# sulaimanvesal/PointCloudUDA

Hardware: AMD Instinct MI355X
Metric: adversarial train-step images/sec (seg+3 discr) at 256x256 (higher is better)
Workload: dtype bf16x3 MFMA (split-bf16, fp32 accumulate; fp32 storage); 1 GPU; MS-CMRSeg full UDA: UNet(PointNet head) + d1 + d2 + d4, 256x256x1, 4 classes; per_gpu_batch=32, global_batch=32, precision=bf16x3, parallelism=dp1, ranks_in_group=1, collective=none, streams=discriminators concurrent, d_target_forward=replayed from the adversarial pass of the same step, launch=eager (256 host cores for this rank)

## Files before the change

pointcloududa_amd/csrc/conv_wgrad.hip:

```cpp
#include "conv_igemm.h"
#include "conv_host.h"

struct ReduceJobs {
  int n;
  int first_block[PCUDA_REDUCE_MAX_JOBS + 1];
  pcuda_reduce_job j[PCUDA_REDUCE_MAX_JOBS];
};

__global__ __launch_bounds__(1024) void wgrad_reduce_batch_kernel(const ReduceJobs jobs) {
  __shared__ float sh[16][64];
  int lo = 0, hi = jobs.n - 1;
  while (lo < hi) {
    const int mid = (lo + hi + 1) >> 1;
    if (jobs.first_block[mid] <= (int)blockIdx.x) lo = mid; else hi = mid - 1;
  }
  const pcuda_reduce_job& jb = jobs.j[lo];
  const float* partial = jb.partial;
  long long numel = jb.numel;
  float* dw = jb.dw;
  int ntaps = jb.ntaps;
  const int ksplit = jb.ksplit, nkg = jb.nkg;
  const int lane = threadIdx.x & 63, kg = threadIdx.x >> 6;
  const long long nblk_w = (numel + 63) / 64;
  long long blk = (int)blockIdx.x - jobs.first_block[lo];
  if (blk >= nblk_w) { blk -= nblk_w; partial = jb.db_partial; numel = jb.nb; dw = jb.db; ntaps = 1; }
  const long long i = blk * 64 + lane;
  float s = 0.f;
  if (i < numel && kg < nkg) {
    int k = kg;
    for (; k + 7 * nkg < ksplit; k += 8 * nkg) {
      float v[8];
#pragma unroll
      for (int u = 0; u < 8; ++u) v[u] = partial[(long long)(k + u * nkg) * numel + i];
#pragma unroll
      for (int u = 0; u < 8; ++u) s += v[u];
    }
    for (; k < ksplit; k += nkg) s += partial[(long long)k * numel + i];
  }
  sh[kg][lane] = s;
  __syncthreads();
  if (kg == 0 && i < numel) {
    float t = 0.f;
    for (int q = 0; q < nkg; ++q) t += sh[q][lane];
    long long o = i;
    if (ntaps > 1) {
      const long long cc = numel / ntaps;
      const long long tt = i / cc, r = i - tt * cc;
      o = r * ntaps + tt;
    }
    dw[o] = jb.accumulate ? dw[o] + t : t;
  }
}

static int reduce_blocks(const pcuda_reduce_job& jb) { return cdiv(jb.numel, 64) + (jb.db ? cdiv(jb.nb, 64) : 0); }

static int launch_reduce_jobs(const ReduceJobs& jobs, int threads, hipStream_t s) {
  hipLaunchKernelGGL(wgrad_reduce_batch_kernel, dim3(jobs.first_block[jobs.n]), dim3(threads), 0, s, jobs);
  PCUDA_CHECK_LAUNCH("wgrad_reduce_batch_kernel");
  return PCUDA_OK;
}

static pcuda_reduce_job reduce_job(const float* partial, long long numel, int ksplit, float* dw, int accumulate, int ntaps,
                                   const float* db_partial, long long nb, float* db) {
  pcuda_reduce_job jb;
  memset(&jb, 0, sizeof(jb));
  jb.partial = partial; jb.numel = numel; jb.ksplit = ksplit; jb.dw = dw; jb.accumulate = accumulate; jb.ntaps = ntaps;
  jb.db_partial = db_partial; jb.nb = db ? nb : 0; jb.db = db;
  jb.nkg = 1;
  while (jb.nkg < 16 && jb.nkg * 2 <= ksplit) jb.nkg <<= 1;
  return jb;
}

static int launch_reduce_job(const pcuda_reduce_job& jb, hipStream_t s) {
  ReduceJobs jobs;
  jobs.n = 1;
  jobs.j[0] = jb;
  jobs.first_block[0] = 0;
  jobs.first_block[1] = reduce_blocks(jb);
  return launch_reduce_jobs(jobs, 64 * jb.nkg, s);
}
int launch_wgrad_reduce(const float* partial, long long numel, int ksplit, float* dw, int accumulate, int ntaps,
                        const float* db_partial, long long nb, float* db, hipStream_t s) {
  return launch_reduce_job(reduce_job(partial, numel, ksplit, dw, accumulate, ntaps, db_partial, nb, db), s);
}

WgradSlabs wgrad_slabs(const WgradCall& c, int slices, int ntaps) {
  WgradSlabs sl;
  sl.welems = (long long)c.g->cout * c.g->cin * c.g->k * c.g->k;
  sl.partial = (float*)c.workspace;
  sl.db_partial = c.db ? sl.partial + (size_t)slices * sl.welems : nullptr;
  sl.slices = slices; sl.ntaps = ntaps;
  return sl;
}

int wgrad_finish(const WgradCall& c, const WgradSlabs& sl) {
  const pcuda_reduce_job jb = reduce_job(sl.partial, sl.welems, sl.slices, c.dw, c.accumulate, sl.ntaps, sl.db_partial, c.g->cout, c.db);
  if (!c.defer) return launch_reduce_job(jb, c.s);
  *c.defer = jb;
  return PCUDA_OK;
}

extern "C" int pcuda_wgrad_reduce_batch(const pcuda_reduce_job* host_jobs, int njobs, pcuda_stream_t s) {
  if (!host_jobs || njobs < 0) PCUDA_FAIL(PCUDA_E_BADARG, "wgrad_reduce_batch: bad arguments");
  int done = 0;
  while (done < njobs) {
    ReduceJobs jobs;
    jobs.n = 0;
    int blocks = 0;
    for (; done < njobs && jobs.n < PCUDA_REDUCE_MAX_JOBS; ++done) {
      const pcuda_reduce_job& jb = host_jobs[done];
      if (jb.ksplit <= 0) continue;
      if (!jb.partial || !jb.dw || jb.numel <= 0 || jb.nkg < 1 || jb.nkg > 16 || (jb.db && !jb.db_partial))
        PCUDA_FAIL(PCUDA_E_BADARG, "wgrad_reduce_batch: bad job %d", done);
      jobs.first_block[jobs.n] = blocks;
      jobs.j[jobs.n++] = jb;
      blocks += reduce_blocks(jb);
    }
    if (jobs.n == 0) break;
    jobs.first_block[jobs.n] = blocks;
    ProfScope prof(PCUDA_FAM_POINTWISE, 0.0, (hipStream_t)s, "wgrad reduce batch");
    const int rc = launch_reduce_jobs(jobs, 1024, (hipStream_t)s);
    if (rc) return rc;
  }
  return PCUDA_OK;
}

namespace {

struct WgradPlan {
  int co_blks, co_tile, n_co_tiles, n_chunks, tap_groups, taps_per_group, tw, th, tiles_x, tiles_y, ksplit;
  int ih_t, iw_t;
};

struct TileSpan {
  long long halo, clipped;
};
TileSpan tile_span(const pcuda_conv_geom* g, long long ih, long long iw) {
  return {ih * iw, (ih < g->in_h ? ih : g->in_h) * (iw < g->in_w ? iw : g->in_w) + 1};
}
size_t stage_lds(long long x_pixels, int co_tile, size_t mul) {
  return (size_t)x_pixels * IG_REC_BYTES * mul + (size_t)co_tile * WG_ZROW * mul;
}

struct WgradStage {
  bool clamp;
  int x_cap;
  size_t lds;
};
WgradStage wgrad_stage(const WgradPlan& w, const pcuda_conv_geom* g, size_t mul) {
  const TileSpan t = tile_span(g, w.ih_t, w.iw_t);
  WgradStage st;
  st.clamp = t.clipped * 2 <= t.halo || stage_lds(t.halo, w.co_tile, mul) > (size_t)LDS_HARD;
  st.x_cap = (int)(st.clamp ? t.clipped : t.halo);
  st.lds = stage_lds(st.x_cap, w.co_tile, mul);
  return st;
}

WgradPlan plan_wgrad(const pcuda_conv_geom* g) {
  WgradPlan w;
  w.co_blks = ig_co_blks(g->cout);
  w.co_tile = 32 * w.co_blks;
  w.n_co_tiles = cdiv(g->cout, w.co_tile);
  w.n_chunks = cdiv(g->cin, 32);
  const int ntaps = g->k * g->k;
  w.tap_groups = ntaps <= 16 ? 1 : cdiv(ntaps, 9);
  w.taps_per_group = cdiv(ntaps, w.tap_groups);
  const int span = (g->k - 1) * g->dil;
  {
    int cand[16];
    const int nc = tile_width_candidates(g->out_w, 128, cand);
    long long best_key = -1;
    w.tw = 32; w.th = 4;
    for (int ci = 0; ci < nc; ++ci) {
      const int tw = cand[ci], th = 128 / tw;
      if (th < 1) continue;
      const TileSpan t = tile_span(g, (th - 1) * g->stride + span + 1, (tw - 1) * g->stride + span + 1);
      const long long cap = t.halo < t.clipped ? t.halo : t.clipped;
      if (stage_lds(cap, w.co_tile, 2) > (size_t)LDS_HARD) continue;
      const long long staged = (t.clipped * 2 <= t.halo) ? t.clipped : t.halo;
      const long long key = ((long long)cdiv(g->out_w, tw) * cdiv(g->out_h, th) << 24) + (staged > 768 ? (1ll << 22) : 0) +
                            ((tw & 31) ? (1ll << 20) : 0) + t.halo;
      if (best_key < 0 || key < best_key) { best_key = key; w.tw = tw; w.th = th; }
    }
  }
  const int TW = w.tw, TH = w.th;
  w.tiles_x = cdiv(g->out_w, TW);
  w.tiles_y = cdiv(g->out_h, TH);
  w.ih_t = (TH - 1) * g->stride + span + 1;
  w.iw_t = (TW - 1) * g->stride + span + 1;
  const long long ntiles = (long long)g->n * w.tiles_x * w.tiles_y;
  const int base = w.n_co_tiles * w.n_chunks * w.tap_groups;
  static const int tgt32 = env_knob("PCUDA_WG_BLOCKS32", 768);
  static const int tgt64 = env_knob("PCUDA_WG_BLOCKS64", 1024);
  static const int tgt1 = env_knob("PCUDA_WG_BLOCKS1", 256);
  const bool one_per_cu = wgrad_stage(w, g, 2).lds > (size_t)LDS_HARD / 2;
  long long ks = (one_per_cu ? tgt1 : (w.co_blks == 1 ? tgt32 : tgt64)) / base;
  if (ks < 1) ks = 1;
  if (ks > ntiles) ks = ntiles;
  const long long welems = (long long)g->cout * g->cin * ntaps;
  while (ks > 1 && ks * welems * 4 > (64ll << 20)) ks >>= 1;
  if (ks >= 8) ks &= ~7ll;
  w.ksplit = (int)ks;
  return w;
}

int wgrad_prefetch(const WgradCall& c, const WgradPlan& w, int x_cap) {
  static const bool nopipe = env_knob("PCUDA_NOPIPE", 0) != 0;
  int pf = (nopipe || !fast_src_ok(c.x, c.g->cin)) ? 0 : (x_cap <= 256 ? 1 : (x_cap <= 768 ? 3 : 0));
  static const bool now8 = env_knob("PCUDA_WG_NO8", 0) != 0;
  if (!now8 && pf > 0 && w.taps_per_group > 9 && x_cap <= 1024) pf = 100 + (x_cap <= 512 ? 1 : 2);
  return pf;
}

WgradParams wgrad_params(const WgradCall& c, const WgradPlan& w, const TapSet& t, const WgradStage& st, int pf, const dim3& grid) {
  const pcuda_conv_geom* g = c.g;
  WgradParams p;
  memset(&p, 0, sizeof(p));
  p.x = *c.x; p.cin = g->cin;
  p.in_h = g->in_h; p.in_w = g->in_w; p.in_shift = g->in_up ? 1 : 0; p.in_row = g->in_w >> p.in_shift;
  p.dz = c.dy; p.dz_sn = c.dy_sn; p.dz_sc = c.dy_sc;
  p.cout = g->cout; p.out_h = g->out_h; p.out_w = g->out_w;
  p.stride = g->stride;
  p.ntaps = w.taps_per_group; p.ntaps_total = t.n; p.tap_groups = w.tap_groups;
  memcpy(p.dy, t.dy, sizeof(p.dy));
  memcpy(p.dx, t.dx, sizeof(p.dx));
  p.dy_min = t.dy_min; p.dx_min = t.dx_min;
  p.ih_t = w.ih_t; p.iw_t = w.iw_t;
  p.tw = w.tw; p.th = w.th; p.tmagic = 65536 / w.tw + 1; p.tiles_x = w.tiles_x; p.tiles_y = w.tiles_y; p.n = g->n;
  p.ksplit = w.ksplit; p.n_co_tiles = w.n_co_tiles; p.n_chunks = w.n_chunks;
  p.partial = (float*)c.workspace;
  static const int dbg = env_knob("PCUDA_DBG", 0);
  p.dbg = dbg;
  p.tw16 = ((w.tw & 15) == 0 && w.tw * w.th == 128) ? 1 : 0;
  p.aligned4 = ((g->out_w & 7) == 0 && (w.tw & 7) == 0 && aligned16(c.dy, c.dy_sn, c.dy_sc) &&
                ((long long)g->cout * c.dy_sc + (long long)g->out_h * g->out_w) * 4 < (1ll << 30)) ? 1 : 0;
  static const bool noxcd = env_knob("PCUDA_WG_NOXCD", 0) != 0;
  static const bool nointer = env_knob("PCUDA_WG_NOINTER", 0) != 0;
  const long long nblk = (long long)grid.x * grid.y;
  p.xcd_items = (!noxcd && nblk >= 16 && (nblk & 7) == 0) ? (int)(nblk / 8) : 0;
  p.xcd_slices = (p.xcd_items && !nointer && (w.ksplit & 7) == 0) ? w.ksplit / 8 : 0;
  {
    static const bool noxq = env_knob("PCUDA_NOXQ", 0) != 0;
    const int slots = pf >= 100 ? pf - 100 : pf, per = pf >= 100 ? 128 : 64;
    const int ih = st.clamp ? (w.ih_t < g->in_h ? w.ih_t : g->in_h) : w.ih_t;
    const int in_w_phys = g->in_up ? g->in_w / 2 : g->in_w;
    p.xq = (!noxq && slots > 0 && !g->in_up && (in_w_phys & 3) == 0 && (ih * ((w.iw_t + 6) / 4) + per - 1) / per <= slots) ? 1 : 0;
  }
  return p;
}

}

int wgrad_dispatch_x3(const WgradParams& p, int co_blks, bool clamp, int taps_max, int pf, int x_cap, size_t lds,
                      float* dbp, dim3 grid, hipStream_t s);
int wgrad_dispatch_bf16(const WgradParams& p, int co_blks, bool clamp, int taps_max, int pf, int x_cap, size_t lds,
                        float* dbp, dim3 grid, hipStream_t s);

static int generic_slices(const pcuda_conv_geom* g) { return plan_wgrad(g).ksplit; }
static int generic_wgrad(const WgradCall& c) {
  const pcuda_conv_geom* g = c.g;
  const bool x3 = c.prec == PCUDA_PREC_BF16X3;
  const WgradPlan w = plan_wgrad(g);
  const TapSet t = fwd_taps(g);
  const WgradSlabs sl = wgrad_slabs(c, w.ksplit, t.n);
  const WgradStage st = wgrad_stage(w, g, x3 ? 2 : 1);
  if (st.lds > (size_t)LDS_HARD) PCUDA_FAIL(PCUDA_E_UNSUPPORTED, "conv2d_wgrad: tile %dx%d does not fit LDS", w.ih_t, w.iw_t);
  const dim3 grid(w.n_co_tiles * w.n_chunks * w.tap_groups, w.ksplit);
  const int pf = wgrad_prefetch(c, w, st.x_cap);
  const WgradParams p = wgrad_params(c, w, t, st, pf, grid);
  {
    const double flops = 2.0 * g->n * (double)g->out_h * g->out_w * g->cout * (double)g->cin * t.n;
    char tag[160];
    snprintf(tag, sizeof(tag), "wgrad n%d cin%d cout%d %dx%d k%d s%d d%d ksplit%d clamp%d pf%d lds%zu", g->n, g->cin,
             g->cout, g->out_h, g->out_w, g->k, g->stride, g->dil, w.ksplit, st.clamp ? 1 : 0, pf, st.lds);
    ProfScope prof(PCUDA_FAM_CONV_WGRAD, flops, c.s, tag);
    const int taps_max = w.taps_per_group <= 1 ? 1 : w.taps_per_group <= 9 ? 9 : 16;
    const int rc = x3 ? wgrad_dispatch_x3(p, w.co_blks, st.clamp, taps_max, pf, st.x_cap, st.lds, sl.db_partial, grid, c.s)
                      : wgrad_dispatch_bf16(p, w.co_blks, st.clamp, taps_max, pf, st.x_cap, st.lds, sl.db_partial, grid, c.s);
    if (rc) return rc;
  }
  return wgrad_finish(c, sl);
}

struct WgradRoute {
  const char* name;
  int (*slices)(const pcuda_conv_geom* g);
  size_t (*bytes)(const pcuda_conv_geom* g);
  int (*run)(const WgradCall& c);
};
static const WgradRoute WGRAD_ROUTES[] = {
    {"direct c1", direct_wgrad_slices, nullptr, direct_wgrad},
    {"direct d1", nullptr, direct_d1_wgrad_bytes, direct_d1_wgrad},
    {"wgrad3r", wgrad3r_slices, nullptr, wgrad3r_wgrad},
    {"wgrad3", wgrad3_slices, nullptr, wgrad3_wgrad},
    {"wgrad1", wgrad1_slices, nullptr, wgrad1_wgrad},
    {"generic", generic_slices, nullptr, generic_wgrad},
};

extern "C" size_t pcuda_conv2d_wgrad_workspace_size(const pcuda_conv_geom* g) {
  if (!geom_ok(g)) return 0;
  size_t need = 0;
  for (const WgradRoute& r : WGRAD_ROUTES) {
    size_t b = 0;
    if (r.bytes) b = r.bytes(g);
    else if (const int slices = r.slices(g)) b = wgrad_slab_bytes(g, slices);
    if (b > need) need = b;
  }
  return need;
}

static int wgrad_impl(const WgradCall& c, size_t workspace_bytes) {
  const pcuda_conv_geom* g = c.g;
  if (!geom_ok(g)) PCUDA_FAIL(PCUDA_E_BADARG, "conv2d_wgrad: inconsistent geometry");
  if (!src_ok(c.x, g->cin) || !c.dy || !c.dw) PCUDA_FAIL(PCUDA_E_BADARG, "conv2d_wgrad: bad tensors");
  if (c.prec != PCUDA_PREC_BF16X3 && c.prec != PCUDA_PREC_BF16) PCUDA_FAIL(PCUDA_E_BADARG, "conv2d_wgrad: bad precision");
  if (!c.workspace || workspace_bytes < pcuda_conv2d_wgrad_workspace_size(g))
    PCUDA_FAIL(PCUDA_E_WORKSPACE, "conv2d_wgrad: workspace too small (%zu < %zu)", workspace_bytes,
               pcuda_conv2d_wgrad_workspace_size(g));
  for (const WgradRoute& r : WGRAD_ROUTES) {
    const int rc = r.run(c);
    if (rc != WGRAD_NOT_TAKEN) return rc;
  }
  PCUDA_FAIL(PCUDA_E_UNSUPPORTED, "conv2d_wgrad: no route took the layer");
}

extern "C" int pcuda_conv2d_wgrad(const pcuda_conv_geom* g, int prec, const pcuda_src* x, const float* dy,
                                  long long dy_sn, long long dy_sc, float* dw, float* db, int accumulate,
                                  void* workspace, size_t workspace_bytes, pcuda_stream_t s) {
  return wgrad_impl({g, prec, x, dy, dy_sn, dy_sc, dw, db, accumulate, workspace, (hipStream_t)s, nullptr}, workspace_bytes);
}

extern "C" int pcuda_conv2d_wgrad_partial(const pcuda_conv_geom* g, int prec, const pcuda_src* x, const float* dy,
                                          long long dy_sn, long long dy_sc, float* dw, float* db, int accumulate,
                                          void* workspace, size_t workspace_bytes, pcuda_reduce_job* job, pcuda_stream_t s) {
  if (!job) PCUDA_FAIL(PCUDA_E_BADARG, "conv2d_wgrad_partial: job is NULL");
  memset(job, 0, sizeof(*job));
  return wgrad_impl({g, prec, x, dy, dy_sn, dy_sc, dw, db, accumulate, workspace, (hipStream_t)s, job}, workspace_bytes);
}
```

pointcloududa_amd/csrc/dense.hip:

```cpp
#include "common.h"

struct GemmParams {
  const float* a; long long a_sb, a_si, a_sl;
  const float* b; long long b_sb, b_sl, b_sj;
  float* c; long long c_sb, c_si, c_sj;
  const float* bias;
  int m, n, k, accumulate;
};

#define GT 32
__global__ __launch_bounds__(256) void gemm_kernel(const GemmParams p) {
  __shared__ float As[GT][GT + 1], Bs[GT][GT + 1];
  const int bz = blockIdx.z;
  const float* A = p.a + bz * p.a_sb;
  const float* B = p.b + bz * p.b_sb;
  float* C = p.c + bz * p.c_sb;
  const int i0 = blockIdx.y * GT, j0 = blockIdx.x * GT;
  const int tj = threadIdx.x & 31, ti = threadIdx.x >> 5;
  float acc[4] = {0.f, 0.f, 0.f, 0.f};
  for (int l0 = 0; l0 < p.k; l0 += GT) {
    for (int e = threadIdx.x; e < GT * GT; e += 256) {
      const int r = e >> 5, cc = e & 31;
      int ia, la;
      if (p.a_sl == 1) { ia = r; la = cc; } else { ia = cc; la = r; }
      As[ia][la] = (i0 + ia < p.m && l0 + la < p.k) ? A[(i0 + ia) * p.a_si + (l0 + la) * p.a_sl] : 0.f;
      int lb, jb;
      if (p.b_sj == 1) { lb = r; jb = cc; } else { lb = cc; jb = r; }
      Bs[lb][jb] = (l0 + lb < p.k && j0 + jb < p.n) ? B[(l0 + lb) * p.b_sl + (j0 + jb) * p.b_sj] : 0.f;
    }
    __syncthreads();
#pragma unroll 8
    for (int l = 0; l < GT; ++l) {
      const float bv = Bs[l][tj];
#pragma unroll
      for (int q = 0; q < 4; ++q) acc[q] += As[ti * 4 + q][l] * bv;
    }
    __syncthreads();
  }
  const int j = j0 + tj;
  if (j < p.n) {
    const float bj = p.bias ? p.bias[j] : 0.f;
#pragma unroll
    for (int q = 0; q < 4; ++q) {
      const int i = i0 + ti * 4 + q;
      if (i < p.m) {
        float* dst = C + i * p.c_si + j * p.c_sj;
        const float v = acc[q] + bj;
        *dst = p.accumulate ? *dst + v : v;
      }
    }
  }
}

#define SK_COLS 8
#define SK_WAVES 16
__global__ __launch_bounds__(64 * SK_WAVES) void gemm_skinny_kernel(const GemmParams p) {
  __shared__ float red[SK_WAVES][64][SK_COLS];
  const int lane = threadIdx.x & 63, wv = threadIdx.x >> 6;
  const int j0 = blockIdx.x * SK_COLS;
  const int i = min(lane, p.m - 1);
  const float* arow = p.a + (long long)i * p.a_si;
  const int kq = (p.k + SK_WAVES - 1) / SK_WAVES, l_lo = wv * kq, l_hi = min(p.k, l_lo + kq);
  float acc[SK_COLS];
#pragma unroll
  for (int c = 0; c < SK_COLS; ++c) acc[c] = 0.f;
  const float* bcol[SK_COLS];
#pragma unroll
  for (int c = 0; c < SK_COLS; ++c) bcol[c] = p.b + (long long)min(j0 + c, p.n - 1) * p.b_sj;
#pragma unroll 4
  for (int l = l_lo; l < l_hi; ++l) {
    const float av = arow[(long long)l * p.a_sl];
#pragma unroll
    for (int c = 0; c < SK_COLS; ++c) acc[c] = fmaf(av, bcol[c][(long long)l * p.b_sl], acc[c]);
  }
#pragma unroll
  for (int c = 0; c < SK_COLS; ++c) red[wv][lane][c] = acc[c];
  __syncthreads();
  for (int e = threadIdx.x; e < 64 * SK_COLS; e += 64 * SK_WAVES) {
    const int r = e / SK_COLS, c = e - r * SK_COLS, j = j0 + c;
    if (r < p.m && j < p.n) {
      float v = 0.f;
#pragma unroll
      for (int q = 0; q < SK_WAVES; ++q) v += red[q][r][c];
      v += p.bias ? p.bias[j] : 0.f;
      float* dst = p.c + (long long)r * p.c_si + (long long)j * p.c_sj;
      *dst = p.accumulate ? *dst + v : v;
    }
  }
}


__global__ __launch_bounds__(256) void colsum_kernel(const float* __restrict__ dy, int m, int n, float* db,
                                                     int accumulate, int cp) {
  __shared__ float sh[256];
  const int rparts = 256 / cp;
  const int c = threadIdx.x % cp, rp = threadIdx.x / cp;
  const int j = blockIdx.x * cp + c;
  float s = 0.f;
  if (j < n)
    for (int i = rp; i < m; i += rparts) s += dy[(long long)i * n + j];
  sh[threadIdx.x] = s;
  __syncthreads();
  for (int half = rparts >> 1; half > 0; half >>= 1) {
    if (rp < half) sh[threadIdx.x] += sh[threadIdx.x + half * cp];
    __syncthreads();
  }
  if (rp == 0 && j < n) db[j] = accumulate ? db[j] + sh[c] : sh[c];
}

__global__ void splitk_reduce_kernel(const float* __restrict__ part, long long numel, int ksplit,
                                     float* __restrict__ out, int accumulate) {
  for (long long i = blockIdx.x * (long long)blockDim.x + threadIdx.x; i < numel;
       i += (long long)gridDim.x * blockDim.x) {
    float s = 0.f;
    for (int k = 0; k < ksplit; ++k) s += part[(long long)k * numel + i];
    out[i] = accumulate ? out[i] + s : s;
  }
}

__global__ __launch_bounds__(256) void max_points_fwd_kernel(const float* __restrict__ x, int rows, int l,
                                                             float* __restrict__ y, int* __restrict__ idx) {
  const int row = blockIdx.x * 4 + (threadIdx.x >> 6), lane = threadIdx.x & 63;
  if (row >= rows) return;
  const float* p = x + (long long)row * l;
  float best = -INFINITY;
  int bi = 0x7fffffff;
  for (int i = lane; i < l; i += 64) {
    const float v = p[i];
    if (v > best) { best = v; bi = i; }
  }
#pragma unroll
  for (int o = 32; o > 0; o >>= 1) {
    const float ov = __shfl_xor(best, o, 64);
    const int oi = __shfl_xor(bi, o, 64);
    if (ov > best || (ov == best && oi < bi)) { best = ov; bi = oi; }
  }
  if (lane == 0) { y[row] = best; idx[row] = bi; }
}

__global__ __launch_bounds__(256) void max_points_bwd_kernel(const float* __restrict__ dy, const int* __restrict__ idx,
                                                             int rows, int l, float* __restrict__ dx) {
  const long long total = (long long)rows * l;
  for (long long e = blockIdx.x * 256ll + threadIdx.x; e < total; e += 256ll * gridDim.x) {
    const int row = (int)(e / l), i = (int)(e - (long long)row * l);
    dx[e] = (idx[row] == i) ? dy[row] : 0.f;
  }
}

namespace {
int launch_gemm(const GemmParams& p, int batch, hipStream_t s) {
  if (p.m <= 0 || p.n <= 0 || p.k <= 0 || batch <= 0) PCUDA_FAIL(PCUDA_E_BADARG, "gemm: bad dims");
  if (batch == 1 && p.m <= 64 && p.k >= 64) {
    hipLaunchKernelGGL(gemm_skinny_kernel, dim3(cdiv(p.n, SK_COLS)), dim3(64 * SK_WAVES), 0, s, p);
    PCUDA_CHECK_LAUNCH("gemm_skinny_kernel");
    return PCUDA_OK;
  }
  dim3 grid(cdiv(p.n, GT), cdiv(p.m, GT), batch);
  hipLaunchKernelGGL(gemm_kernel, grid, dim3(256), 0, s, p);
  PCUDA_CHECK_LAUNCH("gemm_kernel");
  return PCUDA_OK;
}
}

extern "C" int pcuda_linear_fwd(const float* x, const float* w, const float* b, float* y, int m, int k, int n,
                                pcuda_stream_t s) {
  if (!x || !w || !y) PCUDA_FAIL(PCUDA_E_BADARG, "linear_fwd: null pointer");
  GemmParams p = {x, 0, k, 1, w, 0, 1, k, y, 0, n, 1, b, m, n, k, 0};
  return launch_gemm(p, 1, (hipStream_t)s);
}

extern "C" int pcuda_linear_bwd_x(const float* dy, const float* w, float* dx, int m, int k, int n, int accumulate,
                                  pcuda_stream_t s) {
  if (!dy || !w || !dx) PCUDA_FAIL(PCUDA_E_BADARG, "linear_bwd_x: null pointer");
  GemmParams p = {dy, 0, n, 1, w, 0, k, 1, dx, 0, k, 1, nullptr, m, k, n, accumulate};
  return launch_gemm(p, 1, (hipStream_t)s);
}

extern "C" size_t pcuda_linear_bwd_w_workspace_size(int m, int k, int n) {
  const long long out_elems = (long long)n * k;
  if (m >= 2048 && out_elems <= 65536) {
    int ks = m / 256;
    if (ks > 64) ks = 64;
    return (size_t)(ks + 1) * out_elems * sizeof(float);
  }
  return 0;
}

extern "C" int pcuda_linear_bwd_w(const float* dy, const float* x, float* dw, float* db, int m, int k, int n,
                                  int accumulate, void* workspace, size_t workspace_bytes, pcuda_stream_t s) {
  if (!dy || !x || !dw) PCUDA_FAIL(PCUDA_E_BADARG, "linear_bwd_w: null pointer");
  const long long out_elems = (long long)n * k;
  const size_t need = pcuda_linear_bwd_w_workspace_size(m, k, n);
  int rc;
  if (need > 0 && workspace && workspace_bytes >= need) {
    float* slab = (float*)workspace;
    int ks = m / 256;
    if (ks > 64) ks = 64;
    const int mk = (m + ks - 1) / ks;
    const int full = m / mk;
    GemmParams pb = {dy, (long long)mk * n, 1, n, x, (long long)mk * k, k, 1, slab, out_elems, k, 1, nullptr, n, k, mk, 0};
    rc = launch_gemm(pb, full, (hipStream_t)s);
    if (rc) return rc;
    int nsl = full;
    if (m - full * mk > 0) {
      GemmParams pt = {dy + (long long)full * mk * n, 0, 1, n, x + (long long)full * mk * k, 0, k, 1,
                       slab + (long long)full * out_elems, 0, k, 1, nullptr, n, k, m - full * mk, 0};
      rc = launch_gemm(pt, 1, (hipStream_t)s);
      if (rc) return rc;
      ++nsl;
    }
    hipLaunchKernelGGL(splitk_reduce_kernel, dim3(cdiv(out_elems, 256)), dim3(256), 0, (hipStream_t)s,
                       (const float*)slab, out_elems, nsl, dw, accumulate);
    PCUDA_CHECK_LAUNCH("splitk_reduce_kernel");
  } else {
    GemmParams p = {dy, 0, 1, n, x, 0, k, 1, dw, 0, k, 1, nullptr, n, k, m, accumulate};
    rc = launch_gemm(p, 1, (hipStream_t)s);
    if (rc) return rc;
  }
  if (db) {
    int cp = 1;
    while (cp < n && cp < 64) cp <<= 1;
    hipLaunchKernelGGL(colsum_kernel, dim3(cdiv(n, cp)), dim3(256), 0, (hipStream_t)s, dy, m, n, db, accumulate, cp);
    PCUDA_CHECK_LAUNCH("colsum_kernel");
  }
  return PCUDA_OK;
}

extern "C" int pcuda_bmm(const float* a, const float* bmat, float* c, int batch, int m, int k, int n, int ta, int tb,
                         int accumulate, pcuda_stream_t s) {
  if (!a || !bmat || !c) PCUDA_FAIL(PCUDA_E_BADARG, "bmm: null pointer");
  GemmParams p;
  p.a = a; p.a_sb = (long long)m * k; p.a_si = ta ? 1 : k; p.a_sl = ta ? m : 1;
  p.b = bmat; p.b_sb = (long long)k * n; p.b_sl = tb ? 1 : n; p.b_sj = tb ? k : 1;
  p.c = c; p.c_sb = (long long)m * n; p.c_si = n; p.c_sj = 1;
  p.bias = nullptr; p.m = m; p.n = n; p.k = k; p.accumulate = accumulate;
  return launch_gemm(p, batch, (hipStream_t)s);
}

extern "C" int pcuda_max_points_fwd(const float* x, int b, int c, int l, float* y, int* idx, pcuda_stream_t s) {
  if (!x || !y || !idx || b <= 0 || c <= 0 || l <= 0) PCUDA_FAIL(PCUDA_E_BADARG, "max_points_fwd: bad arguments");
  const int rows = b * c;
  hipLaunchKernelGGL(max_points_fwd_kernel, dim3(cdiv(rows, 4)), dim3(256), 0, (hipStream_t)s, x, rows, l, y, idx);
  PCUDA_CHECK_LAUNCH("max_points_fwd_kernel");
  return PCUDA_OK;
}

extern "C" int pcuda_max_points_bwd(const float* dy, const int* idx, int b, int c, int l, float* dx, pcuda_stream_t s) {
  if (!dy || !idx || !dx || b <= 0 || c <= 0 || l <= 0) PCUDA_FAIL(PCUDA_E_BADARG, "max_points_bwd: bad arguments");
  const long long total = (long long)b * c * l;
  const int blocks = (int)(cdiv(total, 256) > 4096 ? 4096 : cdiv(total, 256));
  hipLaunchKernelGGL(max_points_bwd_kernel, dim3(blocks), dim3(256), 0, (hipStream_t)s, dy, idx, b * c, l, dx);
  PCUDA_CHECK_LAUNCH("max_points_bwd_kernel");
  return PCUDA_OK;
}
```

Baseline: 762.9 img/s.

## Rewrite wgrad split-K reduce with vectorized loads and LDS-transposed coalesced stores

Replaces the wgrad split-K reduction kernel with a tiled version. Each 256-thread workgroup handles a block of rows across all taps, loads partials as float4 with several independent accumulators, and reduces the k-groups in shared memory. The tap transpose is staged through an LDS tile so dw writes are contiguous and vectorized, where the old kernel scattered them through the (r*ntaps+tt) remap. It also unrolls the dense split-K reduce loop by 8. The new code adds index arithmetic with magic divisors, a limit on the number of taps, and more shared memory per block, which may lower occupancy.

Measured after the change: 767.7 img/s, median of 6. No clear change (+0.6%).

```diff
diff --git a/pointcloududa_amd/csrc/conv_wgrad.hip b/pointcloududa_amd/csrc/conv_wgrad.hip
--- a/pointcloududa_amd/csrc/conv_wgrad.hip
+++ b/pointcloududa_amd/csrc/conv_wgrad.hip
@@ -1,61 +1,17 @@
 #include "conv_igemm.h"
 #include "conv_host.h"
 
-struct ReduceJobs {
-  int n;
-  int first_block[PCUDA_REDUCE_MAX_JOBS + 1];
-  pcuda_reduce_job j[PCUDA_REDUCE_MAX_JOBS];
-};
-
-__global__ __launch_bounds__(1024) void wgrad_reduce_batch_kernel(const ReduceJobs jobs) {
-  __shared__ float sh[16][64];
-  int lo = 0, hi = jobs.n - 1;
-  while (lo < hi) {
-    const int mid = (lo + hi + 1) >> 1;
-    if (jobs.first_block[mid] <= (int)blockIdx.x) lo = mid; else hi = mid - 1;
-  }
-  const pcuda_reduce_job& jb = jobs.j[lo];
-  const float* partial = jb.partial;
-  long long numel = jb.numel;
-  float* dw = jb.dw;
-  int ntaps = jb.ntaps;
-  const int ksplit = jb.ksplit, nkg = jb.nkg;
-  const int lane = threadIdx.x & 63, kg = threadIdx.x >> 6;
-  const long long nblk_w = (numel + 63) / 64;
-  long long blk = (int)blockIdx.x - jobs.first_block[lo];
-  if (blk >= nblk_w) { blk -= nblk_w; partial = jb.db_partial; numel = jb.nb; dw = jb.db; ntaps = 1; }
-  const long long i = blk * 64 + lane;
-  float s = 0.f;
-  if (i < numel && kg < nkg) {
-    int k = kg;
-    for (; k + 7 * nkg < ksplit; k += 8 * nkg) {
-      float v[8];
-#pragma unroll
-      for (int u = 0; u < 8; ++u) v[u] = partial[(long long)(k + u * nkg) * numel + i];
-#pragma unroll
-      for (int u = 0; u < 8; ++u) s += v[u];
-    }
-    for (; k < ksplit; k += nkg) s += partial[(long long)k * numel + i];
-  }
-  sh[kg][lane] = s;
-  __syncthreads();
-  if (kg == 0 && i < numel) {
-    float t = 0.f;
-    for (int q = 0; q < nkg; ++q) t += sh[q][lane];
-    long long o = i;
-    if (ntaps > 1) {
-      const long long cc = numel / ntaps;
-      const long long tt = i / cc, r = i - tt * cc;
-      o = r * ntaps + tt;
-    }
-    dw[o] = jb.accumulate ? dw[o] + t : t;
-  }
-}
-
-static int reduce_blocks(const pcuda_reduce_job& jb) { return cdiv(jb.numel, 64) + (jb.db ? cdiv(jb.nb, 64) : 0); }
-
-static int launch_reduce_jobs(const ReduceJobs& jobs, int threads, hipStream_t s) {
-  hipLaunchKernelGGL(wgrad_reduce_batch_kernel, dim3(jobs.first_block[jobs.n]), dim3(threads), 0, s, jobs);
+#define RED_SYNC() __syncthreads()
+#include "wgrad_reduce.h"
+
+__global__ __launch_bounds__(RED_T, 4) void wgrad_reduce_batch_kernel(const ReduceJobs jobs) {
+  __shared__ __attribute__((aligned(16))) float sc[RED_T * RED_U * 4];
+  __shared__ __attribute__((aligned(16))) float tile[RED_TILE];
+  red_workgroup(jobs, (int)blockIdx.x, (int)threadIdx.x, sc, tile);
+}
+
+static int launch_reduce_jobs(const ReduceJobs& jobs, hipStream_t s) {
+  hipLaunchKernelGGL(wgrad_reduce_batch_kernel, dim3(jobs.first_block[jobs.n]), dim3(RED_T), 0, s, jobs);
   PCUDA_CHECK_LAUNCH("wgrad_reduce_batch_kernel");
   return PCUDA_OK;
 }
@@ -76,8 +32,8 @@
   jobs.n = 1;
   jobs.j[0] = jb;
   jobs.first_block[0] = 0;
-  jobs.first_block[1] = reduce_blocks(jb);
-  return launch_reduce_jobs(jobs, 64 * jb.nkg, s);
+  jobs.first_block[1] = (int)reduce_blocks(jb);
+  return launch_reduce_jobs(jobs, s);
 }
 int launch_wgrad_reduce(const float* partial, long long numel, int ksplit, float* dw, int accumulate, int ntaps,
                         const float* db_partial, long long nb, float* db, hipStream_t s) {
@@ -110,16 +66,17 @@
     for (; done < njobs && jobs.n < PCUDA_REDUCE_MAX_JOBS; ++done) {
       const pcuda_reduce_job& jb = host_jobs[done];
       if (jb.ksplit <= 0) continue;
-      if (!jb.partial || !jb.dw || jb.numel <= 0 || jb.nkg < 1 || jb.nkg > 16 || (jb.db && !jb.db_partial))
+      if (!jb.partial || !jb.dw || jb.numel <= 0 || jb.nkg < 1 || jb.nkg > 16 || (jb.db && !jb.db_partial) || jb.ntaps < 1 ||
+          jb.ntaps > RED_MAX_TAPS || jb.numel % jb.ntaps)
         PCUDA_FAIL(PCUDA_E_BADARG, "wgrad_reduce_batch: bad job %d", done);
       jobs.first_block[jobs.n] = blocks;
       jobs.j[jobs.n++] = jb;
-      blocks += reduce_blocks(jb);
+      blocks += (int)reduce_blocks(jb);
     }
     if (jobs.n == 0) break;
     jobs.first_block[jobs.n] = blocks;
     ProfScope prof(PCUDA_FAM_POINTWISE, 0.0, (hipStream_t)s, "wgrad reduce batch");
-    const int rc = launch_reduce_jobs(jobs, 1024, (hipStream_t)s);
+    const int rc = launch_reduce_jobs(jobs, (hipStream_t)s);
     if (rc) return rc;
   }
   return PCUDA_OK;
diff --git a/pointcloududa_amd/csrc/dense.hip b/pointcloududa_amd/csrc/dense.hip
--- a/pointcloududa_amd/csrc/dense.hip
+++ b/pointcloududa_amd/csrc/dense.hip
@@ -113,7 +113,15 @@
   for (long long i = blockIdx.x * (long long)blockDim.x + threadIdx.x; i < numel;
        i += (long long)gridDim.x * blockDim.x) {
     float s = 0.f;
-    for (int k = 0; k < ksplit; ++k) s += part[(long long)k * numel + i];
+    int k = 0;
+    for (; k + 8 <= ksplit; k += 8) {
+      float v[8];
+#pragma unroll
+      for (int u = 0; u < 8; ++u) v[u] = part[(long long)(k + u) * numel + i];
+#pragma unroll
+      for (int u = 0; u < 8; ++u) s += v[u];
+    }
+    for (; k < ksplit; ++k) s += part[(long long)k * numel + i];
     out[i] = accumulate ? out[i] + s : s;
   }
 }
diff --git a/pointcloududa_amd/csrc/wgrad_reduce.h b/pointcloududa_amd/csrc/wgrad_reduce.h
--- /dev/null
+++ b/pointcloududa_amd/csrc/wgrad_reduce.h
@@ -0,0 +1,182 @@
+#pragma once
+#include <stdint.h>
+#include "../../include/pcuda_hip.h"
+
+#ifdef __HIPCC__
+#define RED_HD __host__ __device__ inline
+#define RED_D __device__ __forceinline__
+typedef float4 red_f4;
+#else
+#define RED_HD inline
+#define RED_D inline
+struct alignas(16) red_f4 { float x, y, z, w; };
+#endif
+
+struct ReduceJobs {
+  int n;
+  int first_block[PCUDA_REDUCE_MAX_JOBS + 1];
+  pcuda_reduce_job j[PCUDA_REDUCE_MAX_JOBS];
+};
+
+constexpr int RED_T = 256;
+constexpr int RED_U = 4;
+constexpr int RED_TILE = 4608;
+constexpr int RED_MIN_ROWS = 32;
+constexpr int RED_MAX_TAPS = RED_TILE / RED_MIN_ROWS;
+
+RED_HD int reduce_rows(long long cc, int ntaps) {
+  int r = RED_MIN_ROWS;
+  while (2 * r * ntaps <= RED_TILE) r *= 2;
+  while (r > RED_MIN_ROWS && (cc + r - 1) / r < 1024) r >>= 1;
+  return r;
+}
+
+RED_HD long long reduce_blocks(const pcuda_reduce_job& jb) {
+  const long long cc = jb.numel / jb.ntaps;
+  const int rw = reduce_rows(cc, jb.ntaps), rb = reduce_rows(jb.nb, 1);
+  return (cc + rw - 1) / rw + (jb.db ? (jb.nb + rb - 1) / rb : 0);
+}
+
+RED_D unsigned red_magic(int d) { return 0xffffffffu / (unsigned)d + 1u; }
+RED_D int red_div(int n, int d, unsigned m) { return d == 1 ? n : (int)(((unsigned long long)(unsigned)n * m) >> 32); }
+
+template <int V>
+RED_D void red_ld(float (&v)[V], const float* p) {
+  if constexpr (V == 4) {
+    const red_f4 t = *reinterpret_cast<const red_f4*>(p);
+    v[0] = t.x; v[1] = t.y; v[2] = t.z; v[3] = t.w;
+  } else {
+    v[0] = *p;
+  }
+}
+
+template <int U, int S, int V>
+RED_D void red_sum(const float* const (&p)[RED_U], const bool (&last)[RED_U], int full, bool ragged, long long stride,
+                   float (&s)[RED_U][V]) {
+  int j = 0;
+  for (; j + S <= full; j += S) {
+    float v[S][U][V];
+#pragma unroll
+    for (int jj = 0; jj < S; ++jj)
+#pragma unroll
+      for (int u = 0; u < U; ++u) red_ld<V>(v[jj][u], p[u] + (j + jj) * stride);
+#pragma unroll
+    for (int jj = 0; jj < S; ++jj)
+#pragma unroll
+      for (int u = 0; u < U; ++u)
+#pragma unroll
+        for (int e = 0; e < V; ++e) s[u][e] += v[jj][u][e];
+  }
+  for (; j < full; ++j) {
+    float v[U][V];
+#pragma unroll
+    for (int u = 0; u < U; ++u) red_ld<V>(v[u], p[u] + j * stride);
+#pragma unroll
+    for (int u = 0; u < U; ++u)
+#pragma unroll
+      for (int e = 0; e < V; ++e) s[u][e] += v[u][e];
+  }
+  if (!ragged) return;
+  float v[U][V];
+#pragma unroll
+  for (int u = 0; u < U; ++u) red_ld<V>(v[u], last[u] ? p[u] + full * stride : p[u]);
+#pragma unroll
+  for (int u = 0; u < U; ++u)
+#pragma unroll
+    for (int e = 0; e < V; ++e) s[u][e] = last[u] ? s[u][e] + v[u][e] : s[u][e];
+}
+
+template <int V>
+RED_D void red_block(const float* partial, long long cc, int ntaps, int ksplit, int nkg, float* dw, int accumulate, long long r0,
+                     int rb, int tid, float* sc, float* tile) {
+  const long long numel = cc * ntaps, stride = (long long)nkg * numel;
+  const int cpt = rb / V, ncol = cpt * ntaps;
+  const int full = ksplit / nkg;
+  const int npass = (ncol * nkg + RED_T * RED_U - 1) / (RED_T * RED_U), pc_fit = RED_T * RED_U / nkg;
+  const int pc_max = (ncol + npass - 1) / npass < pc_fit ? (ncol + npass - 1) / npass : pc_fit;
+  const unsigned m_cpt = red_magic(cpt);
+  for (int c0 = 0; c0 < ncol; c0 += pc_max) {
+    const int pc = pc_max < ncol - c0 ? pc_max : ncol - c0, nt = pc * nkg;
+    const unsigned m_pc = red_magic(pc);
+    const float* p[RED_U];
+    bool last[RED_U];
+    float s[RED_U][V];
+    int nu = 0;
+#pragma unroll
+    for (int u = 0; u < RED_U; ++u) {
+      const int t = tid + u * RED_T;
+      const bool live = t < nt;
+      nu += live;
+      const int q = live ? red_div(t, pc, m_pc) : 0, c = c0 + (live ? t - q * pc : 0);
+      const int tap = red_div(c, cpt, m_cpt), rv = c - tap * cpt;
+      p[u] = partial + (q < ksplit ? q : 0) * numel + tap * cc + r0 + rv * V;
+      last[u] = live && q + (long long)full * nkg < ksplit;
+#pragma unroll
+      for (int e = 0; e < V; ++e) s[u][e] = 0.f;
+    }
+    if (nu > 2) red_sum<4, 2, V>(p, last, full, ksplit % nkg != 0, stride, s);
+    else if (nu == 2) red_sum<2, 4, V>(p, last, full, ksplit % nkg != 0, stride, s);
+    else if (nu == 1) red_sum<1, 8, V>(p, last, full, ksplit % nkg != 0, stride, s);
+#pragma unroll
+    for (int u = 0; u < RED_U; ++u) {
+      const int t = tid + u * RED_T;
+      if (t < nt) {
+        if constexpr (V == 4) *reinterpret_cast<red_f4*>(sc + 4 * t) = red_f4{s[u][0], s[u][1], s[u][2], s[u][3]};
+        else sc[t] = s[u][0];
+      }
+    }
+    RED_SYNC();
+    for (int cl = tid; cl < pc; cl += RED_T) {
+      float t[V];
+#pragma unroll
+      for (int e = 0; e < V; ++e) t[e] = 0.f;
+#pragma unroll 4
+      for (int q = 0; q < nkg; ++q) {
+        float v[V];
+        red_ld<V>(v, sc + V * (q * pc + cl));
+#pragma unroll
+        for (int e = 0; e < V; ++e) t[e] += v[e];
+      }
+      const int c = c0 + cl, tap = red_div(c, cpt, m_cpt), rv = c - tap * cpt;
+#pragma unroll
+      for (int e = 0; e < V; ++e) tile[(rv * V + e) * ntaps + tap] = t[e];
+    }
+    RED_SYNC();
+  }
+  float* out = dw + r0 * ntaps;
+  const int n = rb * ntaps;
+  if constexpr (V == 4) {
+    for (int i = tid; i < n / 4; i += RED_T) {
+      red_f4 t = *reinterpret_cast<const red_f4*>(tile + 4 * i);
+      if (accumulate) {
+        const red_f4 d = *reinterpret_cast<const red_f4*>(out + 4 * i);
+        t.x = d.x + t.x; t.y = d.y + t.y; t.z = d.z + t.z; t.w = d.w + t.w;
+      }
+      *reinterpret_cast<red_f4*>(out + 4 * i) = t;
+    }
+  } else {
+    for (int i = tid; i < n; i += RED_T) out[i] = accumulate ? out[i] + tile[i] : tile[i];
+  }
+}
+
+RED_D void red_workgroup(const ReduceJobs& jobs, int block, int tid, float* sc, float* tile) {
+  int lo = 0, hi = jobs.n - 1;
+  while (lo < hi) {
+    const int mid = (lo + hi + 1) >> 1;
+    if (jobs.first_block[mid] <= block) lo = mid; else hi = mid - 1;
+  }
+  const pcuda_reduce_job& jb = jobs.j[lo];
+  const float* partial = jb.partial;
+  float* dw = jb.dw;
+  int ntaps = jb.ntaps;
+  long long cc = jb.numel / ntaps;
+  int rows = reduce_rows(cc, ntaps);
+  long long blk = block - jobs.first_block[lo];
+  const long long nblk_w = (cc + rows - 1) / rows;
+  if (blk >= nblk_w) { blk -= nblk_w; partial = jb.db_partial; cc = jb.nb; dw = jb.db; ntaps = 1; rows = reduce_rows(cc, 1); }
+  const long long r0 = blk * rows;
+  const int rb = (int)(rows < cc - r0 ? rows : cc - r0);
+  const bool vec = cc % 4 == 0 && (((uintptr_t)partial | (uintptr_t)dw) & 15) == 0;
+  if (vec) red_block<4>(partial, cc, ntaps, jb.ksplit, jb.nkg, dw, jb.accumulate, r0, rb, tid, sc, tile);
+  else red_block<1>(partial, cc, ntaps, jb.ksplit, jb.nkg, dw, jb.accumulate, r0, rb, tid, sc, tile);
+}
```
